# WoodOxen/tactics2d

Measured on NVIDIA H100. Metric: participant_steps_per_sec, higher is better.
Workload: dtype f32

## Files before the change

include/t2d_b200.h:

```cpp
#ifndef T2D_B200_H
#define T2D_B200_H

#include <stdint.h>

#ifdef __cplusplus
extern "C" {
#endif

#define T2D_VERSION 100

#define T2D_OK 0
#define T2D_E_INVALID (-1)
#define T2D_E_CUDA (-2)
#define T2D_E_UNSUPPORTED (-3)
#define T2D_E_STATE (-4)

#define T2D_MODEL_KINEMATICS 0
#define T2D_MODEL_DYNAMICS 1
#define T2D_MODEL_POINTMASS_NEWTON 2
#define T2D_MODEL_POINTMASS_EULER 3
#define T2D_MODEL_STATIC 4
#define T2D_MODEL_DRIFT 5

#define T2D_SHAPE_OBB 0
// ... 258 lines not shown
                        uint8_t* agent_status, float* iou, uint8_t* done, float* max_iou, float* min_dist,
                        uint8_t* traffic_status, int reset_trackers_on_done, void* stream);

int t2d_scatter_agent_action(t2d_ctx* ctx, const int16_t* observers , int32_t n_observers,
                             const float* agent_action , float* action ,
                             void* stream);
int t2d_step_host_agents(t2d_ctx* ctx, const float* agent_action_host , float* action ,
                         uint8_t* flags, int16_t* hit_index, int16_t* hit_segment, float* max_iou, float* min_dist,
                         int reset_trackers_on_done, float* reward_host, uint8_t* terminated_host, uint8_t* truncated_host,
                         uint8_t* agent_status_host, uint8_t* done_host, void* stream);

typedef struct t2d_exchange t2d_exchange;
int t2d_exchange_create(t2d_exchange** out, int device, int world, int rank, int n_local, int slots, void* ipc_handle_out);
int t2d_exchange_connect(t2d_exchange* x, const void* handles );
int t2d_exchange_allgather(t2d_exchange* x, const uint8_t* done_local, uint8_t* dst, void* stream);
int t2d_exchange_allgather_lagged(t2d_exchange* x, const uint8_t* done_local, uint8_t* dst, int lag, void* stream);
int t2d_exchange_status(t2d_exchange* x, uint32_t* steps, uint32_t* timed_out);
int t2d_exchange_destroy(t2d_exchange* x);

int t2d_physics_step(int device, const t2d_type_params* params , int interval_ms, int delta_t_ms, int n,
                     float* x, float* y, float* heading, float* speed, float* vx, float* vy, float* omega_front,
                     float* omega_rear, const float* action, float* applied, void* stream);

int t2d_set_prefetch(t2d_ctx* ctx, int mode);

int64_t t2d_launch_count(void);

int64_t t2d_tick_fixed_count(void);

int64_t t2d_tick_order_fallback_count(void);

int t2d_order_hint(t2d_ctx* ctx, void* read_to, const void* write_from);

int64_t t2d_tick_instance_count(int k);

#ifdef __cplusplus
}
#endif
#endif
```

tactics2d_b200/_lib.py:

```python

from __future__ import annotations

import ctypes as C
import os

_HERE = os.path.dirname(os.path.abspath(__file__))
LIB_PATH = os.environ.get("T2D_B200_LIB", os.path.join(_HERE, "libt2d_b200.so"))


class T2DError(RuntimeError):
    """A C-ABI call returned a negative code; the message is ``t2d_last_error()``."""


class Config(C.Structure):
    _fields_ = [("interval_ms", C.c_int32), ("delta_t_ms", C.c_int32), ("max_step", C.c_int32),
                ("flags", C.c_int32)]


class TypeParamsC(C.Structure):
    _fields_ = [(n, C.c_float) for n in (
        "half_len", "half_wid", "radius", "lf", "lr", "steer_lo", "steer_hi", "speed_lo", "speed_hi",
        "accel_lo", "accel_hi", "mass", "mass_height", "mu", "I_z", "cf", "cr")] + [
        ("model", C.c_int32), ("shape", C.c_int32)] + [(n, C.c_float) for n in ("wheel_radius", "T_sb", "T_se", "I_yw")]

# ... 81 lines not shown
    "t2d_bev_render_agents": (C.c_int, [_P, _P, C.c_int32, _P, C.c_int, C.c_int, _P, C.c_int, _P, _P]),
    "t2d_observe": (C.c_int, [_P, C.POINTER(ObsConfigC), _P, _P, _P, _P]),
    "t2d_observe_agents": (C.c_int, [_P, C.POINTER(ObsConfigC), _P, C.c_int32, _P, _P, _P, _P, _P]),
    "t2d_set_controllers": (C.c_int, [_P, _P, C.c_int, _P, _P, _P, _P]),
    "t2d_set_paths": (C.c_int, [_P, _P, _P, C.c_int]),
    "t2d_control": (C.c_int, [_P, _P, _P]),
    "t2d_set_pid": (C.c_int, [_P, _P, _P]),
    "t2d_set_leader_search": (C.c_int, [_P, C.c_double, C.c_double, _P, _P]),
    "t2d_find_leaders": (C.c_int, [_P, C.c_double, C.c_double, _P, _P, _P]),
    "t2d_set_lane_change": (C.c_int, [_P, _P, _P, _P, _P, _P, _P]),
    "t2d_set_routes": (C.c_int, [_P, _P, C.c_double, C.c_double, C.c_float]),
    "t2d_bind_route_trackers": (C.c_int, [_P, _P, _P, C.c_int32]),
    "t2d_route_observe": (C.c_int, [_P, _P, C.c_int32, C.c_int, C.c_float, _P, _P]),
    "t2d_set_history": (C.c_int, [_P, C.c_int32]),
    "t2d_observe_history": (C.c_int, [_P, _P, C.c_int32, _P, C.c_int32, _P, _P]),
    "t2d_history_view": (C.c_int, [_P, C.POINTER(HistoryRingC)]),
    "t2d_exchange_create": (C.c_int, [C.POINTER(_P), C.c_int, C.c_int, C.c_int, C.c_int, C.c_int, _P]),
    "t2d_exchange_connect": (C.c_int, [_P, _P]),
    "t2d_exchange_allgather": (C.c_int, [_P, _P, _P, _P]),
    "t2d_exchange_allgather_lagged": (C.c_int, [_P, _P, _P, C.c_int, _P]),
    "t2d_exchange_status": (C.c_int, [_P, C.POINTER(C.c_uint32), C.POINTER(C.c_uint32)]),
    "t2d_exchange_destroy": (C.c_int, [_P]),
    "t2d_physics_step": (C.c_int, [C.c_int, C.POINTER(TypeParamsC), C.c_int, C.c_int, C.c_int] + [_P] * 11),
    "t2d_bind_wheel_state": (C.c_int, [_P, _P, _P]),
    "t2d_bind_reset_wheel_pool": (C.c_int, [_P, _P, _P]),
    "t2d_set_log": (C.c_int, [_P, C.POINTER(LogC)]),
    "t2d_set_log_schedule": (C.c_int, [_P, C.POINTER(LogC), _P, _P, C.c_int32, _P]),
    "t2d_set_log_reactive": (C.c_int, [_P, C.POINTER(ReactiveReplayC)]),
    "t2d_set_prefetch": (C.c_int, [_P, C.c_int]),
    "t2d_launch_count": (C.c_int64, []),
    "t2d_tick_fixed_count": (C.c_int64, []),
    "t2d_tick_order_fallback_count": (C.c_int64, []),
    "t2d_order_hint": (C.c_int, [_P, _P, _P]),
    "t2d_tick_instance_count": (C.c_int64, [C.c_int]),
}

_lib = None


def load():
    global _lib
    if _lib is not None:
        return _lib
    if not os.path.exists(LIB_PATH):
        raise ImportError(
            f"{LIB_PATH} not found: build it with `python -c 'import __graft_entry__ as g; g.build()'` "
            "(nvcc -gencode arch=compute_90a,code=sm_90a).  tactics2d_b200 has no CPU fallback.")
    lib = C.CDLL(LIB_PATH)
    for name, (res, args) in SYMBOLS.items():
        fn = getattr(lib, name)
        fn.restype = res
        fn.argtypes = args
    _lib = lib
    return lib


def check(code: int):
    if code != 0:
        msg = load().t2d_last_error()
        raise T2DError(f"t2d error {code}: {msg.decode() if msg else ''}")
```

tactics2d_b200/csrc/t2d_kernels.cu:

```cuda
#include <cuda_runtime.h>
#include <stddef.h>
#include <stdint.h>
#include <stdio.h>
#include <string.h>

#include <algorithm>
#include <atomic>
#include <cmath>
#include <memory>
#include <mutex>
#include <string>
#include <vector>

#include "../../include/t2d_b200.h"
#include "t2d_math.cuh"
#include "t2d_world.cuh"
#include "t2d_tick.cuh"
#include "t2d_reset.cuh"
#include "t2d_route.cuh"
#include "t2d_agents.cuh"
#include "t2d_replay.cuh"
#include "t2d_lidar.cuh"
#include "t2d_exchange.cuh"
#include "t2d_control.cuh"
// ... 195 lines not shown
  float* ctrl_last_accel = nullptr;
  bool ctrl_has_pid = false;
  bool ctrl_pid_reads_target = false;
  const float* pid_target = nullptr;
  double* pid_state = nullptr;
  dev_ptr<PathVertex> d_path_v;
  dev_ptr<int> d_path_off;
  int n_paths = 0;
  int16_t* leader_lead = nullptr;
  float* leader_gap = nullptr;
  double leader_half_width = 0.0, leader_max_range = 0.0;
  std::unique_ptr<LaneChange> lane;
  std::unique_ptr<ReactiveReplay> reactive;
  const int16_t* route_id = nullptr;
  double route_threshold = 0.0, route_weight = 0.0;
  float route_off_reward = 0.0f;
  double* route_s_best = nullptr;
  double* route_agent_s_best = nullptr;
  int route_agent_rows = 0;
  std::unique_ptr<ChunkedUpload> hs_upload;
  Mirror hs_out;
  MappedEgo hs_ego;
  AgentStaging ha;
  dev_ptr<uint8_t> ha_flags;
  int host_chunks = 0;
  int n_bev_styles = 0;
  t2d_bev_style bev_style[bev::MAX_STYLES] = {};
  uint8_t bev_type_style[T2D_MAX_TYPES] = {};
  int bev_target_style = bev::NO_STYLE;
  std::unique_ptr<DeviceLog> log;
  std::vector<int> type_model;
  std::vector<t2d_type_params> type_rows;
  dev_ptr<uint8_t> order;
  std::unique_ptr<DeviceSampler> sampler;
  std::unique_ptr<DeviceHistory> hist;
};

enum : unsigned { NEED_STATE = 1, NEED_TABLE = 2, NEED_TICK = 4 };

static int require(const t2d_ctx* c, unsigned need) {
  if ((need & NEED_STATE) && !c->x) return fail(T2D_E_STATE, "state not bound: call t2d_bind_state first");
  if ((need & NEED_TABLE) && (!c->d_table || c->n_types == 0))
    return fail(T2D_E_STATE, "type table not set: call t2d_set_type_table first");
  if (need & NEED_TICK) {
    if (c->has_drift && !(c->wheel_f && c->wheel_r))
      return fail(T2D_E_STATE, "the type table holds a SingleTrackDrift row: call t2d_bind_wheel_state first");
    if (c->log && c->log->type_id != c->type_id) return fail(T2D_E_STATE, "state rebound after t2d_set_log: call t2d_set_log again");
  }
  return T2D_OK;
}

static WorldArgs world_args(const t2d_ctx* c) {
  return {c->x, c->y, c->h, c->v, c->vx, c->vy, c->type_id, c->step_count, c->d_table.get(), c->n_types, c->N, c->M};
}

static RouteArgs route_args(const t2d_ctx* c) {
  return {c->route_id, c->d_path_v.get(), c->d_path_off.get(), c->n_paths, c->route_off_reward, c->route_threshold,
          c->route_weight};
}

static int check_route_trackers(const t2d_ctx* c, const char* fn) {
  if (c->route_id && c->route_agent_s_best && c->route_agent_rows != c->agent_q)
    return fail(T2D_E_STATE, std::string(fn) + ": the agents' route tracker has another row count than the bound agents: "
                                               "call t2d_bind_route_trackers again");
  return T2D_OK;
}
// ... 42 lines not shown
  g_launches.fetch_add(1);
  CUDA_TRY(cudaGetLastError());
  return T2D_OK;
}

static int capped_grid(long long items, int per_cta, int sm_count, int per_sm) {
  return (int)std::max(1LL, std::min((items + per_cta - 1) / per_cta, (long long)sm_count * per_sm));
}

static int launch_history(t2d_ctx* c, const uint8_t* mask, void* stream) {
  if (!c->hist) return T2D_OK;
  hist::AppendArgs A{world_args(c)};
  A.ring = history_ring(c); A.track_now = history_track_now(c); A.mask = mask;
  hist::t2d_history_append_kernel<<<(c->N + hist::K15_WARPS - 1) / hist::K15_WARPS, hist::K15_WARPS * 32, 0, (cudaStream_t)stream>>>(A);
  return launched();
}

template <class Args> static void set_time_step(Args& A, int interval_ms, int delta_t_ms) {
  const int delta_t = std::min(delta_t_ms, interval_ms);
  A.n_steps = interval_ms / delta_t;
  A.dt = (float)((double)delta_t / 1000.0);
  A.dt_rem = (float)((double)(interval_ms % delta_t) / 1000.0);
  A.dt_d = (double)delta_t / 1000.0;
  A.dt_rem_d = (double)(interval_ms % delta_t) / 1000.0;
  A.interval_d = (double)interval_ms / 1000.0;
}

extern "C" {

int t2d_version(void) { return T2D_VERSION; }
const char* t2d_last_error(void) { return g_err.c_str(); }
int64_t t2d_launch_count(void) { return (int64_t)g_launches.load(); }
int64_t t2d_tick_fixed_count(void) { return (int64_t)(g_tick_instances[4].load() + g_tick_instances[5].load()); }
int64_t t2d_tick_order_fallback_count(void) {
  std::lock_guard<std::mutex> lock(g_order_mutex);
  int64_t sum = 0;
  for (unsigned long long* d : g_order_fallbacks) {
    if (!d) continue;
    unsigned long long n[ORDER_COUNTERS * ORDER_COUNTER_STRIDE];
    if (cudaMemcpy(n, d, sizeof(n), cudaMemcpyDeviceToHost) != cudaSuccess) return -1;
    for (int i = 0; i < ORDER_COUNTERS; ++i) sum += (int64_t)n[i * ORDER_COUNTER_STRIDE];
  }
  return sum;
}
int64_t t2d_tick_instance_count(int k) { return k >= 0 && k < 7 ? (int64_t)g_tick_instances[k].load() : -1; }

#ifdef T2D_TICK_TIMELINE
int t2d_tick_timeline(void* dst, int64_t bytes, int clear) {
  if (!dst || bytes != (int64_t)sizeof(t2d_timeline)) return fail(T2D_E_INVALID, "timeline buffer size");
  CUDA_TRY(cudaMemcpyFromSymbol(dst, t2d_timeline, sizeof(t2d_timeline)));
  if (clear) {
    void* p = nullptr;
    CUDA_TRY(cudaGetSymbolAddress(&p, t2d_timeline));
    CUDA_TRY(cudaMemset(p, 0, sizeof(t2d_timeline)));
  }
  return T2D_OK;
}
#endif

static int check_cfg(const t2d_config* cfg) {
  if (!cfg) return fail(T2D_E_INVALID, "cfg is NULL");
  if (cfg->interval_ms <= 0) return fail(T2D_E_INVALID, "interval_ms must be > 0");
  if (cfg->delta_t_ms <= 0) return fail(T2D_E_INVALID, "delta_t_ms must be > 0");
  return T2D_OK;
}

int t2d_create(t2d_ctx** out, int device, int n_scenarios, int m_participants, const t2d_config* cfg) {
  if (!out) return fail(T2D_E_INVALID, "out is NULL");
  *out = nullptr;
  if (int r = check_cfg(cfg)) return r;
  if (n_scenarios <= 0 || m_participants <= 0) return fail(T2D_E_INVALID, "n_scenarios and m_participants must be > 0");
  if (m_participants > T2D_MAX_PARTICIPANTS)
    return fail(T2D_E_UNSUPPORTED, "m_participants > 128: a scenario must fit one warp (4 participants per lane)");
  int count = 0;
  CUDA_TRY(cudaGetDeviceCount(&count));
  if (device < 0 || device >= count) return fail(T2D_E_INVALID, "no such CUDA device");
  CUDA_TRY(cudaSetDevice(device));
  t2d_ctx* c = new t2d_ctx();
  c->device = device;
  c->N = n_scenarios;
  c->M = m_participants;
  if (const char* e = getenv("T2D_PDL")) c->use_pdl = atoi(e) != 0;
  if (const char* e = getenv("T2D_GRID_LIMIT")) c->grid_limit = std::max(0, atoi(e));
  if (const char* e = getenv("T2D_TICK_GENERIC")) c->tick_generic = atoi(e) != 0;
  if (const char* e = getenv("T2D_PREFETCH")) c->prefetch_override = atoi(e) != 0 ? 1 : 0;
  if (const char* e = getenv("T2D_WPC")) {
    const int v = atoi(e);
    if (v >= 1 && v <= MAX_WARPS_PER_CTA) c->wpc_override = v;
  }
  if (const char* e = getenv("T2D_HOST_CHUNKS")) c->host_chunks = std::max(0, std::min(atoi(e), MAX_HOST_CHUNKS));
  int g = 1;
  while (g * PPL < m_participants) g <<= 1;
  c->G = g;
  c->cfg = *cfg;
  cudaDeviceProp prop;
  CUDA_TRY(cudaGetDeviceProperties(&prop, device));
  c->sm_count = prop.multiProcessorCount;
  c->max_smem_optin = (int)prop.sharedMemPerBlockOptin;
  {
    std::lock_guard<std::mutex> lock(g_order_mutex);
    unsigned long long*& counters = g_order_fallbacks[device % 64];
    const size_t bytes = ORDER_COUNTERS * ORDER_COUNTER_STRIDE * sizeof(unsigned long long);
    if (!counters && (cudaMalloc(&counters, bytes) != cudaSuccess || cudaMemset(counters, 0, bytes) != cudaSuccess)) {
      cudaFree(counters);
      counters = nullptr;
      delete c;
      return fail(T2D_E_CUDA, "t2d_create: cannot allocate the order fallback counters");
    }
  }
  {
    std::vector<uint8_t> identity((size_t)n_scenarios * FIX_M);
    for (size_t i = 0; i < identity.size(); ++i) identity[i] = (uint8_t)(i % FIX_M);
    if (int r = upload(c->order, identity.data(), identity.size())) {
      delete c;
      return r;
    }
  }
  *out = c;
  return T2D_OK;
}

int t2d_order_hint(t2d_ctx* c, void* read_to, const void* write_from) {
  if (!c) return fail(T2D_E_INVALID, "ctx is NULL");
  CUDA_TRY(cudaSetDevice(c->device));
  const size_t bytes = (size_t)c->N * FIX_M;
  if (read_to) CUDA_TRY(cudaMemcpy(read_to, c->order.get(), bytes, cudaMemcpyDeviceToHost));
  if (write_from) CUDA_TRY(cudaMemcpy(c->order.get(), write_from, bytes, cudaMemcpyHostToDevice));
  return T2D_OK;
}

int t2d_destroy(t2d_ctx* c) {
  if (!c) return T2D_OK;
  cudaSetDevice(c->device);
  delete c;
  return T2D_OK;
}

int t2d_set_config(t2d_ctx* c, const t2d_config* cfg) {
  if (!c) return fail(T2D_E_INVALID, "ctx is NULL");
  if (int r = check_cfg(cfg)) return r;
  c->cfg = *cfg;
  return T2D_OK;
}

int t2d_set_type_table(t2d_ctx* c, const t2d_type_params* table, int n_types) {
  if (!c || !table) return fail(T2D_E_INVALID, "ctx/table is NULL");
  if (n_types <= 0 || n_types > T2D_MAX_TYPES) return fail(T2D_E_INVALID, "n_types must be in 1..64");
  static_assert(sizeof(t2d_type_params) == sizeof(AbiParams), "type table layout");
  if (c->log)
    for (uint8_t row : c->log->track_type_host)
      if (row >= n_types || table[row].model != T2D_MODEL_STATIC)
        return fail(T2D_E_INVALID, "type table: row " + std::to_string(row) + " of a replayed track must exist and be T2D_MODEL_STATIC");
  bool has_pointmass = false, has_drift = false, kin_only = true;
  float rb_max = 0.0f;
  for (int i = 0; i < n_types; ++i) {
    const t2d_type_params& p = table[i];
    if (p.shape == T2D_SHAPE_OBB) rb_max = std::max(rb_max, sqrtf(p.half_len * p.half_len + p.half_wid * p.half_wid) * 1.000002f);
    if (p.shape == T2D_SHAPE_CIRCLE) rb_max = std::max(rb_max, p.radius);
    if (p.model < 0 || p.model > T2D_MODEL_DRIFT) return fail(T2D_E_INVALID, "type table: unknown model id");
    if (p.shape < 0 || p.shape > T2D_SHAPE_NONE) return fail(T2D_E_INVALID, "type table: unknown shape id");
// ... 438 lines not shown
  const int resident_warps = 14;
  if (tiles > (long long)sm_count * resident_warps) return MAX_WARPS_PER_CTA;
  int best = 2;
  double best_cost = 1e30;
  for (int w = 2; w <= MAX_WARPS_PER_CTA; ++w) {
    const long long ctas = (tiles + w - 1) / w;
    const long long per_sm = (ctas + sm_count - 1) / sm_count;
    const double cost = (double)(per_sm * w) + 0.42 * (double)per_sm;
    if (cost < best_cost - 1e-9 || (cost < best_cost + 1e-9 && w > best)) { best_cost = cost; best = w; }
  }
  return best;
}

static int launch_step(t2d_ctx* c, const float* action, const float* ego, uint8_t* flags, int16_t* hit_index, int16_t* hit_segment,
                       uint8_t* scn_status, uint8_t* done, void* stream, int do_physics, int first = 0, int count = -1) {
  if (!c) return fail(T2D_E_INVALID, "ctx is NULL");
  if (int r = require(c, NEED_STATE | NEED_TABLE)) return r;
  if (do_physics && !action) return fail(T2D_E_INVALID, "action is NULL");
  if (do_physics)
    if (int r = require(c, NEED_TICK)) return r;
  CUDA_TRY(cudaSetDevice(c->device));
  if (count < 0) count = c->N - first;
  if (first < 0 || count <= 0 || first + count > c->N) return fail(T2D_E_INVALID, "scenario range out of bounds");
  const DeviceMap& map = c->map;
  const size_t p0 = (size_t)first * c->M;
  StepArgs A{};
  A.x = c->x + p0; A.y = c->y + p0; A.h = c->h + p0; A.v = c->v + p0; A.vx = c->vx + p0; A.vy = c->vy + p0;
  A.type_id = c->type_id + p0; A.step_count = c->step_count + first;
  A.wheel_f = c->wheel_f ? c->wheel_f + p0 : nullptr; A.wheel_r = c->wheel_r ? c->wheel_r + p0 : nullptr;
  A.action = action; A.ego_action = ego ? ego + 2 * (size_t)first : nullptr; A.flags = flags; A.hit_index = hit_index; A.hit_segment = hit_segment;
  A.scn_status = scn_status; A.done = done;
  A.order = c->order.get() + (size_t)first * FIX_M;
  A.order_fallbacks = g_order_fallbacks[c->device % 64];
  const bool map_table = map.n_tiles > 1;
  const MapArgs mp = map_args(map, first);
  A.map_blob = mp.map_blob; A.tile_off = mp.tile_off; A.tile_id = mp.tile_id; A.map_bytes = map.smem_bytes; A.mh = map.mh;
  A.map_in_smem = (!map_table && map.blob && map.mh.n_seg > 0 && map.smem_bytes <= MAP_SMEM_LIMIT) ? 1 : 0;
  A.table = c->d_table.get(); A.n_types = c->n_types;
  A.N = count; A.M = c->M; A.G = c->G;
  set_time_step(A, c->cfg.interval_ms, c->cfg.delta_t_ms);
  A.max_step = c->cfg.max_step; A.cfg_flags = c->cfg.flags;
  A.do_physics = do_physics; A.has_bounds = map.has_bounds ? 1 : 0;
  A.bxmin = map.mh.bxmin; A.bxmax = map.mh.bxmax; A.bymin = map.mh.bymin; A.bymax = map.mh.bymax;
  A.prefetch = c->prefetch_override >= 0 ? c->prefetch_override : (g_exchanges_alive.load() == 0 ? 1 : 0);
  A.needs_vel_in = (c->has_pointmass || c->has_drift || (do_physics && c->log)) ? 1 : 0;
  bool vec = (c->M % PPL == 0) && aligned16(A.x) && aligned16(A.y) && aligned16(A.h) && aligned16(A.v) && aligned16(A.vx) &&
             aligned16(A.vy) && aligned4(A.type_id) && aligned16(action) && aligned4(flags) && aligned8(hit_index) &&
             aligned8(hit_segment);
  A.vec_ok = vec ? 1 : 0;

  A.rb_max = c->rb_max;
  A.goal = c->goal;
  if (A.goal.target) {
    A.goal.target += 5 * (size_t)first; A.goal.iou += first; A.goal.last_pose += 4 * (size_t)first; A.goal.noact_count += first;
  }
  const int table_bytes = (((c->n_types + 1) * (int)sizeof(Params) + 15) / 16) * 16;
  const int spw = 32 / c->G;
  const long long tiles = ((long long)count + spw - 1) / spw;
  int wpc = pick_wpc(tiles, c->sm_count);
  if (c->wpc_override > 0) wpc = c->wpc_override;
  {
    int off = (A.map_in_smem ? A.map_bytes : 0) + table_bytes;
    A.off_poseA = off; off += wpc * POSE_PER_WARP * (int)sizeof(float4);
    A.off_poseB = off; off += wpc * POSE_PER_WARP * (int)sizeof(float4);
    A.off_hit = off; off += wpc * POSE_PER_WARP * (int)sizeof(int);
    A.off_queue = off; off += wpc * QCAP * 4;
// ... 1141 lines not shown
```

tactics2d_b200/csrc/t2d_math.cuh:

```cuda
#pragma once

#include <math.h>
#include <string.h>
#include <stdint.h>

#if defined(__CUDACC__)
#define T2D_HD __host__ __device__ __forceinline__
#define T2D_HD_NOINLINE __host__ __device__ __noinline__
#else
#define T2D_HD inline
#define T2D_HD_NOINLINE
#endif

#if defined(__CUDA_ARCH__)
#define T2D_RSQRTF(x) rsqrtf(x)
#else
#define T2D_RSQRTF(x) (1.0f / sqrtf(x))
#endif

namespace t2d {

constexpr int MODEL_KINEMATICS = 0;
constexpr int MODEL_DYNAMICS = 1;
constexpr int MODEL_POINTMASS_NEWTON = 2;
// ... 144 lines not shown
  float x[W], y[W], h[W], v[W];
  float vx[W], vy[W];
  float ch[W], sh[W];
  float acc[W], steer[W];
};

template <int W>
T2D_HD void kinematics_finish(KinIO<W>& io, const Params* const (&p)[W], const float (&c)[W], const float (&s)[W], float (&v)[W],
                              const float (&Sx)[W], const float (&Sy)[W], const float (&Sv)[W], const float (&kdt)[W],
                              const float (&k)[W], const float (&a)[W], const float (&vlo)[W], const float (&vhi)[W], float dt,
                              float dt_rem) {
#pragma unroll
  for (int i = 0; i < W; ++i) {
    float x = fmaf(dt, Sx[i], io.x[i]);
    float y = fmaf(dt, Sy[i], io.y[i]);
    float dphi = kdt[i] * Sv[i];
    if (dt_rem > 0.0f) {
      x = fmaf(dt_rem * v[i], c[i], x);
      y = fmaf(dt_rem * v[i], s[i], y);
      dphi = fmaf(k[i] * dt_rem, v[i], dphi);
      v[i] = clampf(fmaf(a[i], dt_rem, v[i]), vlo[i], vhi[i]);
    }
    float hn = wrap_two_pi(io.h[i] + dphi);
    float sh, ch;
    sincos_core(hn, sh, ch);
    io.x[i] = x; io.y[i] = y; io.h[i] = hn; io.v[i] = v[i];
    io.vx[i] = v[i] * ch;
    io.vy[i] = v[i] * sh;
    io.ch[i] = ch; io.sh[i] = sh;
  }
}

template <int W>
T2D_HD void kinematics_step(KinIO<W>& io, const Params* const (&p)[W], int n_steps, float dt, float dt_rem) {
  float c[W], s[W], w1[W], Sx[W], Sy[W], Sv[W], kdt[W], adt[W], vlo[W], vhi[W], k[W], a[W];
  bool small = true;
  bool lin = n_steps >= 2 && n_steps <= 24;
  float sd[W], cd[W], sp[W], cp[W];
  bool rare = false;
#pragma unroll
  for (int i = 0; i < W; ++i) {
    const Vec4 g0 = params_group(p[i], 0);
    a[i] = clampf(io.acc[i], g0.x, g0.y);
    const float d = clampf(io.steer[i], g0.z, g0.w);
    io.acc[i] = a[i];
    io.steer[i] = d;
    sincos_poly(d, sd[i], cd[i]);
    sincos_core(io.h[i], sp[i], cp[i]);
    rare = rare || !(fabsf(d) <= 0.78f) || !(fabsf(io.h[i]) <= 512.0f);
  }
  if (rare) {
#pragma unroll
    for (int i = 0; i < W; ++i) {
      if (!(fabsf(io.steer[i]) <= 0.78f)) sincos_fast(io.steer[i], &sd[i], &cd[i]);
      if (!(fabsf(io.h[i]) <= 512.0f)) sincos_fast(io.h[i], &sp[i], &cp[i]);
    }
  }
#pragma unroll
  for (int i = 0; i < W; ++i) {
    const Vec4 g1 = params_group(p[i], 1);
    const float tan_d = T2D_FDIV(sd[i], cd[i]);
    const float tb = g1.z * tan_d;
    const float cb = T2D_RSQRTF(fmaf(tb, tb, 1.0f));
    const float sb = tb * cb;
    k[i] = tan_d * cb * g1.w;
    kdt[i] = k[i] * dt;
    adt[i] = a[i] * dt;
    c[i] = cp[i] * cb - sp[i] * sb;
    s[i] = sp[i] * cb + cp[i] * sb;
    vlo[i] = g1.x;
    vhi[i] = g1.y;
    const float w1u = fmaf(a[i], dt, io.v[i]);
    w1[i] = clampf(w1u, vlo[i], vhi[i]);
    const float wlu = fmaf((float)(n_steps - 1), adt[i], w1[i]);
    const float wl = clampf(fmaf((float)(n_steps - 2), adt[i], w1[i]), vlo[i], vhi[i]);
    lin = lin && (w1u == w1[i]) && (wlu >= vlo[i]) && (wlu <= vhi[i]) && (fabsf(kdt[i] * adt[i]) <= 1e-4f);
    const float wmax = fmaxf(fabsf(io.v[i]), fmaxf(fabsf(w1[i]), fabsf(wl)));
    small = small && (fabsf(kdt[i]) * wmax <= 0.25f);
    Sx[i] = 0.0f; Sy[i] = 0.0f; Sv[i] = 0.0f;
  }
#if defined(__CUDA_ARCH__)
  const bool fast = __all_sync(__activemask(), lin && small);
// ... 622 lines not shown
```

tactics2d_b200/csrc/t2d_tick.cuh:

```cuda
#pragma once

#include "t2d_world.cuh"

namespace t2d {

struct StepArgs {
  float *x, *y, *h, *v, *vx, *vy;
  const uint8_t* type_id;
  int32_t* step_count;
  const float* action;
  const float* ego_action;
  uint8_t* flags;
  int16_t* hit_index;
  int16_t* hit_segment;
  uint8_t* scn_status;
  uint8_t* done;
  const unsigned char* map_blob;
  const uint32_t* tile_off;
  const uint16_t* tile_id;
  MapHeader mh;
  const Params* table;
  int map_bytes, map_in_smem;
  int n_types;
  int N, M, G;
  int g_shift, mp_shift, unused1, n_tiles, wpc, table_bytes;
  int off_poseA, off_poseB, off_hit, off_queue, off_sorted, unused0, off_qcount, off_bar;
  int n_steps;
  float dt, dt_rem;
  double dt_d, dt_rem_d, interval_d;
  int max_step, cfg_flags;
  int do_physics, has_bounds, vec_ok, needs_vel_in;
  int prefetch;
  float bxmin, bxmax, bymin, bymax;
  float rb_max;
  GoalArgs goal;
  float *wheel_f, *wheel_r;
  uint8_t* order;
  unsigned long long* order_fallbacks;
};

__device__ __noinline__ void other_model_step(OneIO& io, const Params& p, int n_steps, double dt, double dt_rem, double interval) {
  if (p.model() == MODEL_DYNAMICS) {
    dynamics_step(io, p, n_steps, dt);
  } else if (p.model() == MODEL_POINTMASS_NEWTON) {
    pointmass_newton_step(io, p, interval);
  } else if (p.model() == MODEL_POINTMASS_EULER) {
    pointmass_euler_step(io, p, n_steps, dt, dt_rem);
  } else {
    sincos_fast(io.h, &io.sh, &io.ch);
  }
}

__device__ __forceinline__ unsigned near_fetch(const float ax, const float ay, const float rbound, const MapHeader& mh, const uint8_t* fine,
                                               unsigned& alt) {
  const float r = rbound * 1.0001f + 1e-3f;
  const float fx = (ax - mh.x0) * mh.inv_cell, fy = (ay - mh.y0) * mh.inv_cell;
  const float gxf = (float)mh.gx, gyf = (float)mh.gy;
  const bool inside = fx >= 0.0f && fy >= 0.0f && fx < gxf && fy < gyf;
  const float kf = (float)mh.fine;
  const int nx = mh.gx * mh.fine, ny = mh.gy * mh.fine;
  const float ux = fmaf(inside ? fx : 0.0f, kf, -0.5f), uy = fmaf(inside ? fy : 0.0f, kf, -0.5f);
  int ix = __float_as_int(ux + RINT_MAGIC) - 0x4B400000, iy = __float_as_int(uy + RINT_MAGIC) - 0x4B400000;
  ix = min(max(ix, 0), nx - 1); iy = min(max(iy, 0), ny - 1);
  const unsigned q = (unsigned)__ldg(fine + (size_t)iy * nx + ix);
  const float ox = fmaxf(fmaxf(-fx, fx - gxf), 0.0f), oy = fmaxf(fmaxf(-fy, fy - gyf), 0.0f);
  const unsigned q_out = fmaxf(ox, oy) * mh.cell <= r ? 0u : 255u;
  alt = inside ? 0xffffffffu : q_out;
  return q;
}
__device__ __forceinline__ bool near_decide(unsigned q, unsigned alt, const float rbound) {
  const unsigned v = alt == 0xffffffffu ? q : alt;
// ... 157 lines not shown
      const MapView mv = map_view(t.sec, *t.mh);
      *sm = static_walk_exact(load_pose(poseA, poseB, ti), poseA[pslot(ti)].z, *t.mh, mv.seg, mv.cell_start, mv.items);
    }
    if (t.mh->n_poly > 0) {
      const float4 pa = poseA[pslot(ti)];
      *sm = static_objects(*sm, pa.x, pa.y, *t.mh, t.blob);
    }
  }
  __syncwarp();
}

__device__ __noinline__ bool oob_slow(const float4* poseA, const float4* poseB, int idx, float xmin, float xmax, float ymin, float ymax) {
  const Pose a = load_pose(poseA, poseB, idx);
  int r = out_of_bound_f32(a.x, a.y, a.c, a.s, a.l, a.w, a.w < 0.0f, xmin, xmax, ymin, ymax);
  if (r < 0) r = out_of_bound_f64(a.x, a.y, a.h, a.l, a.w, a.w < 0.0f, xmin, xmax, ymin, ymax) ? 1 : 0;
  return r != 0;
}

constexpr int FIX_M = 64, FIX_G = 16, FIX_G_SHIFT = 4, FIX_MP_SHIFT = 6;

constexpr int COHORT_BAR = 1;
__device__ __forceinline__ void cohort_arrive(int threads) {
  asm volatile("barrier.arrive %0, %1;" ::"n"(COHORT_BAR), "r"(threads) : "memory");
}
__device__ __forceinline__ void cohort_wait(int threads) {
  asm volatile("barrier.sync %0, %1;" ::"n"(COHORT_BAR), "r"(threads) : "memory");
}

#ifndef T2D_ORDER_PASSES
#define T2D_ORDER_PASSES 2
#endif
constexpr int ORDER_COUNTERS = 64, ORDER_COUNTER_STRIDE = 16;

template <bool FIXED>
__device__ __forceinline__ void prefetch_tile_l2(const StepArgs& A, long long i) {
  asm volatile("prefetch.global.L2 [%0];" ::"l"(A.x + i));
  asm volatile("prefetch.global.L2 [%0];" ::"l"(A.y + i));
  asm volatile("prefetch.global.L2 [%0];" ::"l"(A.h + i));
  asm volatile("prefetch.global.L2 [%0];" ::"l"(A.v + i));
  if (FIXED || A.action) asm volatile("prefetch.global.L2 [%0];" ::"l"(A.action + 2 * i));
  asm volatile("prefetch.global.L2 [%0];" ::"l"(A.type_id + i));
  if (FIXED) asm volatile("prefetch.global.L2 [%0];" ::"l"(A.order + i));
  if (!FIXED && A.needs_vel_in) {
    asm volatile("prefetch.global.L2 [%0];" ::"l"(A.vx + i));
    asm volatile("prefetch.global.L2 [%0];" ::"l"(A.vy + i));
  }
}

#ifdef T2D_TICK_TIMELINE
constexpr int TL_POINTS = 9, TL_MAX_WARPS = 4096;
__device__ unsigned long long t2d_timeline[TL_MAX_WARPS][TL_POINTS][2];
#define T2D_TL(k, on, slot, dep)                                                                                    \
  do {                                                                                                              \
    if ((on) && (slot) < TL_MAX_WARPS) {                                                                            \
      unsigned long long g_, c_;                                                                                    \
      asm volatile("mov.u64 %0, %%globaltimer;\n\tmov.u64 %1, %%clock64;" : "=l"(g_), "=l"(c_) : "f"(dep) : "memory"); \
      t2d_timeline[slot][k][0] = g_;                                                                                \
      t2d_timeline[slot][k][1] = c_;                                                                                \
    }                                                                                                               \
  } while (0)
#else
#define T2D_TL(k, on, slot, dep)
#endif

template <bool KIN_ONLY, bool MAP_TABLE, bool FIXED>
__global__ void __launch_bounds__(CTA_THREADS, 2) t2d_step_kernel(const __grid_constant__ StepArgs A) {
  extern __shared__ __align__(128) unsigned char smem[];
  T2D_TL(0, (threadIdx.x & 31) == 0, (int)(blockIdx.x * A.wpc + (threadIdx.x >> 5)), 0.0f);
  const int map_smem_bytes = (!MAP_TABLE && A.map_in_smem) ? A.map_bytes : 0;
  const int table_bytes = A.table_bytes;
  const int wpc = A.wpc;
  unsigned char* s_map = smem;
  Params* s_table = reinterpret_cast<Params*>(smem + map_smem_bytes);
  float4* s_poseA = reinterpret_cast<float4*>(smem + A.off_poseA);
  float4* s_poseB = reinterpret_cast<float4*>(smem + A.off_poseB);
// ... 36 lines not shown
  float4* poseA = s_poseA + warp * POSE_PER_WARP;
  float4* poseB = s_poseB + warp * POSE_PER_WARP;
  int* hitmin = s_hit + warp * POSE_PER_WARP;
  unsigned* queue = s_queue + warp * QCAP;
  int* qcount = s_qcount + warp;
  const int tb = sub * MP, t0 = tb + m0;
  const int mp_shift = K1_SHAPE(mp_shift, FIX_MP_SHIFT);
  float4* sorted = s_sorted + warp * POSE_PER_WARP + tb;
  const int Mh = M >> 1;

  const int n_tiles = A.n_tiles;
  const int tile0 = (int)blockIdx.x * wpc + warp;
  if (cohort_b) cohort_wait(wpc * 32);
  else if (cohorts && tile0 >= n_tiles) cohort_arrive(wpc * 32);
  for (int tile = tile0; tile < n_tiles; tile += (int)gridDim.x * wpc) {
    const long long n = (long long)tile * spw + sub;
    const bool scn_ok = n < A.N;
    int nvalid = scn_ok ? (FIXED ? PPL : min(PPL, M - m0)) : 0;
    if (nvalid < 0) nvalid = 0;
    const long long idx0 = n * M + m0;
#ifdef T2D_TICK_TIMELINE
    const bool tl_on = lane == 0 && tile == (int)blockIdx.x * wpc + warp;
    const int tl_slot = tile;
#endif

    float sx[PPL], sy[PPL], shd[PPL], sv[PPL], svx[PPL], svy[PPL], a0[PPL], a1[PPL];
    int tidv[PPL];
#pragma unroll
    for (int i = 0; i < PPL; ++i) {
      sx[i] = sy[i] = shd[i] = sv[i] = svx[i] = svy[i] = a0[i] = a1[i] = 0.0f;
      tidv[i] = T2D_TYPE_INACTIVE;
    }
    uint32_t hint = 0x03020100u + 0x04040404u * (uint32_t)gl;
    if (nvalid == PPL && K1_SHAPE(vec_ok, 1)) {
      ld_vec<float, PPL>(A.x + idx0, sx);
      ld_vec<float, PPL>(A.y + idx0, sy);
      ld_vec<float, PPL>(A.h + idx0, shd);
      ld_vec<float, PPL>(A.v + idx0, sv);
      uint8_t tb8[PPL];
      ld_vec<uint8_t, PPL>(A.type_id + idx0, tb8);
      if constexpr (FIXED) hint = *reinterpret_cast<const uint32_t*>(A.order + idx0);
#pragma unroll
      for (int i = 0; i < PPL; ++i) tidv[i] = tb8[i];
      if (K1_SHAPE(do_physics, 1)) {
        float2 act[PPL];
        float lo[4], hi[4];
        ld_vec<float, 4>(A.action + 2 * idx0, lo);
        ld_vec<float, 4>(A.action + 2 * idx0 + 4, hi);
        act[0] = make_float2(lo[0], lo[1]); act[1] = make_float2(lo[2], lo[3]);
        act[2] = make_float2(hi[0], hi[1]); act[3] = make_float2(hi[2], hi[3]);
#pragma unroll
        for (int i = 0; i < PPL; ++i) { a0[i] = act[i].x; a1[i] = act[i].y; }
        if (K1_SHAPE(needs_vel_in, 0)) {
          ld_vec<float, PPL>(A.vx + idx0, svx);
          ld_vec<float, PPL>(A.vy + idx0, svy);
        }
      }
    } else {
#pragma unroll
      for (int i = 0; i < PPL; ++i) {
        if (i < nvalid) {
          sx[i] = A.x[idx0 + i]; sy[i] = A.y[idx0 + i]; shd[i] = A.h[idx0 + i]; sv[i] = A.v[idx0 + i];
          tidv[i] = A.type_id[idx0 + i];
          if (K1_SHAPE(do_physics, 1)) {
            a0[i] = A.action[2 * (idx0 + i)]; a1[i] = A.action[2 * (idx0 + i) + 1];
            if (K1_SHAPE(needs_vel_in, 0)) { svx[i] = A.vx[idx0 + i]; svy[i] = A.vy[idx0 + i]; }
          }
        }
      }
    }
    if (cohorts && !cohort_b && tile == tile0) cohort_arrive(wpc * 32);
    {
      const long long n_next = n + (long long)gridDim.x * wpc * spw;
      if (A.prefetch && n_next < A.N && m0 < M) prefetch_tile_l2<FIXED>(A, n_next * M + m0);
// ... 10 lines not shown
    bool active[PPL], kin[PPL];
    const Params* pp[PPL];
    int model[PPL];
    bool lane_all_kin = true, lane_any_kin = false;
#pragma unroll
    for (int i = 0; i < PPL; ++i) {
      active[i] = tidv[i] < A.n_types;
      pp[i] = &s_table[active[i] ? tidv[i] : 0];
      model[i] = pp[i]->model_shape & 0xff;
      kin[i] = active[i] && (model[i] == MODEL_KINEMATICS);
      lane_all_kin = lane_all_kin && kin[i];
      lane_any_kin = lane_any_kin || kin[i];
      ch[i] = 1.0f; sh[i] = 0.0f;
    }
    T2D_TL(2, tl_on, tl_slot, sx[PPL - 1] + sy[PPL - 1] + shd[PPL - 1] + sv[PPL - 1] + a0[PPL - 1] + a1[PPL - 1] + (float)model[PPL - 1]);
    if (A.cfg_flags & T2D_CFG_STEER_FIRST) {
#pragma unroll
      for (int i = 0; i < PPL; ++i)
        if (model[i] <= MODEL_DYNAMICS || model[i] == MODEL_DRIFT) { float t = a0[i]; a0[i] = a1[i]; a1[i] = t; }
    }

    if (K1_SHAPE(do_physics, 1)) {
      if (__any_sync(0xffffffffu, lane_any_kin)) {
        const Params* const null_row = &s_table[A.n_types];
        const Params* pk[PPL];
        KinIO<PPL> io;
#pragma unroll
        for (int i = 0; i < PPL; ++i) {
          pk[i] = kin[i] ? pp[i] : null_row;
          io.x[i] = kin[i] ? sx[i] : 0.0f; io.y[i] = kin[i] ? sy[i] : 0.0f;
          io.h[i] = kin[i] ? shd[i] : 0.0f; io.v[i] = kin[i] ? sv[i] : 0.0f;
          io.acc[i] = kin[i] ? a0[i] : 0.0f; io.steer[i] = kin[i] ? a1[i] : 0.0f;
        }
        kinematics_step<PPL>(io, pk, A.n_steps, A.dt, A.dt_rem);
#pragma unroll
        for (int i = 0; i < PPL; ++i) {
          if (kin[i]) {
            sx[i] = io.x[i]; sy[i] = io.y[i]; shd[i] = io.h[i]; sv[i] = io.v[i];
            svx[i] = io.vx[i]; svy[i] = io.vy[i]; ch[i] = io.ch[i]; sh[i] = io.sh[i];
          }
        }
      }
      if (!lane_all_kin) {
#pragma unroll
        for (int i = 0; i < PPL; ++i) {
          if (active[i] && !kin[i]) {
            if constexpr (!KIN_ONLY) {
              OneIO io;
              io.x = sx[i]; io.y = sy[i]; io.h = shd[i]; io.v = sv[i]; io.vx = svx[i]; io.vy = svy[i];
              io.a0 = a0[i]; io.a1 = a1[i];
              io.ch = 1.0f; io.sh = 0.0f;
              other_model_step(io, *pp[i], A.n_steps, A.dt_d, A.dt_rem_d, A.interval_d);
              sx[i] = io.x; sy[i] = io.y; shd[i] = io.h; sv[i] = io.v; svx[i] = io.vx; svy[i] = io.vy;
              ch[i] = io.ch; sh[i] = io.sh;
            } else {
              sincos_fast(shd[i], &sh[i], &ch[i]);
            }
          }
        }
      }
      bool all_active = true;
#pragma unroll
      for (int i = 0; i < PPL; ++i) all_active = all_active && active[i];
      if (nvalid == PPL && K1_SHAPE(vec_ok, 1) && all_active) {
        st_vec<float, PPL>(A.x + idx0, sx);
        st_vec<float, PPL>(A.y + idx0, sy);
        st_vec<float, PPL>(A.h + idx0, shd);
        st_vec<float, PPL>(A.v + idx0, sv);
        st_vec<float, PPL>(A.vx + idx0, svx);
        st_vec<float, PPL>(A.vy + idx0, svy);
      } else {
#pragma unroll
        for (int i = 0; i < PPL; ++i) {
          if (i < nvalid && active[i]) {
            A.x[idx0 + i] = sx[i]; A.y[idx0 + i] = sy[i]; A.h[idx0 + i] = shd[i]; A.v[idx0 + i] = sv[i];
            A.vx[idx0 + i] = svx[i]; A.vy[idx0 + i] = svy[i];
          }
        }
      }
    } else {
#pragma unroll
      for (int i = 0; i < PPL; ++i) sincos_fast(shd[i], &sh[i], &ch[i]);
    }
    T2D_TL(3, tl_on, tl_slot, sx[0] + sy[PPL - 1] + ch[0] + sh[PPL - 1]);

    float px[PPL], py[PPL], rb[PPL];
    unsigned solid_bits = 0;
#pragma unroll
    for (int i = 0; i < PPL; ++i) {
      const Vec4 g2 = params_group(pp[i], 2);
      const bool sol = active[i] && (__float_as_int(g2.w) >> 8) != SHAPE_NONE;
      solid_bits |= sol ? (1u << i) : 0u;
      rb[i] = g2.z;
      px[i] = sol ? sx[i] : __int_as_float(0x7fc00000);
      py[i] = sy[i];
      poseA[i * 32 + lane] = make_float4(px[i], py[i], rb[i], shd[i]);
      poseB[i * 32 + lane] = make_float4(ch[i], sh[i], g2.x, g2.y);
    }
    if (lane == 0) *qcount = 0;
    __syncwarp();
    const int cnt_in = (K1_SHAPE(do_physics, 1) && gl == 0 && scn_ok) ? A.step_count[n] : 0;

    unsigned near_q[PPL], near_alt[PPL];
#pragma unroll
    for (int i = 0; i < PPL; ++i) { near_q[i] = 255u; near_alt[i] = 255u; }
    const MapHeader* lane_mh = &A.mh;
    const unsigned char* lane_blob = A.map_blob;
    if constexpr (MAP_TABLE) {
      lane_blob = A.map_blob + A.tile_off[scn_ok ? A.tile_id[n] : 0];
// ... 302 lines not shown
```

Baseline: 17.40 billion.

## Cache heading cos/sin across ticks to skip trig on step entry

Adds a per-participant device cache of cos/sin of heading, tagged with the heading value it was computed for, to the fixed-M world. The kinematic step reuses the cached values when the tag matches the current heading and falls back to sincos per lane on a miss, counting misses in a new counter. This is meant to remove one sincos per participant per tick, at the cost of three extra float loads and three extra stores per participant, plus L2 prefetches for them.

```diff
diff --git a/include/t2d_b200.h b/include/t2d_b200.h
--- a/include/t2d_b200.h
+++ b/include/t2d_b200.h
@@ -314,6 +314,10 @@
 
 int t2d_order_hint(t2d_ctx* ctx, void* read_to, const void* write_from);
 
+int64_t t2d_tick_trig_fallback_count(void);
+
+int t2d_heading_trig(t2d_ctx* ctx, void* read_to, const void* write_from);
+
 int64_t t2d_tick_instance_count(int k);
 
 #ifdef __cplusplus
diff --git a/tactics2d_b200/_lib.py b/tactics2d_b200/_lib.py
--- a/tactics2d_b200/_lib.py
+++ b/tactics2d_b200/_lib.py
@@ -137,6 +137,8 @@
     "t2d_tick_fixed_count": (C.c_int64, []),
     "t2d_tick_order_fallback_count": (C.c_int64, []),
     "t2d_order_hint": (C.c_int, [_P, _P, _P]),
+    "t2d_tick_trig_fallback_count": (C.c_int64, []),
+    "t2d_heading_trig": (C.c_int, [_P, _P, _P]),
     "t2d_tick_instance_count": (C.c_int64, [C.c_int]),
 }
 
diff --git a/tactics2d_b200/csrc/t2d_kernels.cu b/tactics2d_b200/csrc/t2d_kernels.cu
--- a/tactics2d_b200/csrc/t2d_kernels.cu
+++ b/tactics2d_b200/csrc/t2d_kernels.cu
@@ -251,6 +251,7 @@
   std::vector<int> type_model;
   std::vector<t2d_type_params> type_rows;
   dev_ptr<uint8_t> order;
+  dev_ptr<float> trig;
   std::unique_ptr<DeviceSampler> sampler;
   std::unique_ptr<DeviceHistory> hist;
 };
@@ -359,17 +360,19 @@
 const char* t2d_last_error(void) { return g_err.c_str(); }
 int64_t t2d_launch_count(void) { return (int64_t)g_launches.load(); }
 int64_t t2d_tick_fixed_count(void) { return (int64_t)(g_tick_instances[4].load() + g_tick_instances[5].load()); }
-int64_t t2d_tick_order_fallback_count(void) {
+static int64_t fixed_fallback_sum(int set) {
   std::lock_guard<std::mutex> lock(g_order_mutex);
   int64_t sum = 0;
   for (unsigned long long* d : g_order_fallbacks) {
     if (!d) continue;
     unsigned long long n[ORDER_COUNTERS * ORDER_COUNTER_STRIDE];
-    if (cudaMemcpy(n, d, sizeof(n), cudaMemcpyDeviceToHost) != cudaSuccess) return -1;
+    if (cudaMemcpy(n, d + set * ORDER_COUNTERS * ORDER_COUNTER_STRIDE, sizeof(n), cudaMemcpyDeviceToHost) != cudaSuccess) return -1;
     for (int i = 0; i < ORDER_COUNTERS; ++i) sum += (int64_t)n[i * ORDER_COUNTER_STRIDE];
   }
   return sum;
 }
+int64_t t2d_tick_order_fallback_count(void) { return fixed_fallback_sum(0); }
+int64_t t2d_tick_trig_fallback_count(void) { return fixed_fallback_sum(1); }
 int64_t t2d_tick_instance_count(int k) { return k >= 0 && k < 7 ? (int64_t)g_tick_instances[k].load() : -1; }
 
 #ifdef T2D_TICK_TIMELINE
@@ -427,7 +430,7 @@
   {
     std::lock_guard<std::mutex> lock(g_order_mutex);
     unsigned long long*& counters = g_order_fallbacks[device % 64];
-    const size_t bytes = ORDER_COUNTERS * ORDER_COUNTER_STRIDE * sizeof(unsigned long long);
+    const size_t bytes = 2 * ORDER_COUNTERS * ORDER_COUNTER_STRIDE * sizeof(unsigned long long);
     if (!counters && (cudaMalloc(&counters, bytes) != cudaSuccess || cudaMemset(counters, 0, bytes) != cudaSuccess)) {
       cudaFree(counters);
       counters = nullptr;
@@ -443,6 +446,15 @@
       return r;
     }
   }
+  if (m_participants == FIX_M) {
+    const size_t plane = (size_t)n_scenarios * FIX_M;
+    std::vector<float> trig(3 * plane, 0.0f);
+    std::fill(trig.begin(), trig.begin() + plane, 1.0f);
+    if (int r = upload(c->trig, trig.data(), trig.size())) {
+      delete c;
+      return r;
+    }
+  }
   *out = c;
   return T2D_OK;
 }
@@ -453,6 +465,16 @@
   const size_t bytes = (size_t)c->N * FIX_M;
   if (read_to) CUDA_TRY(cudaMemcpy(read_to, c->order.get(), bytes, cudaMemcpyDeviceToHost));
   if (write_from) CUDA_TRY(cudaMemcpy(c->order.get(), write_from, bytes, cudaMemcpyHostToDevice));
+  return T2D_OK;
+}
+
+int t2d_heading_trig(t2d_ctx* c, void* read_to, const void* write_from) {
+  if (!c) return fail(T2D_E_INVALID, "ctx is NULL");
+  if (!c->trig) return fail(T2D_E_UNSUPPORTED, "t2d_heading_trig: the world has no heading trig cache (M != 64)");
+  CUDA_TRY(cudaSetDevice(c->device));
+  const size_t bytes = 3 * (size_t)c->N * FIX_M * sizeof(float);
+  if (read_to) CUDA_TRY(cudaMemcpy(read_to, c->trig.get(), bytes, cudaMemcpyDeviceToHost));
+  if (write_from) CUDA_TRY(cudaMemcpy(c->trig.get(), write_from, bytes, cudaMemcpyHostToDevice));
   return T2D_OK;
 }
 
@@ -957,6 +979,11 @@
   A.scn_status = scn_status; A.done = done;
   A.order = c->order.get() + (size_t)first * FIX_M;
   A.order_fallbacks = g_order_fallbacks[c->device % 64];
+  if (c->trig) {
+    const size_t plane = (size_t)c->N * FIX_M, f0 = (size_t)first * FIX_M;
+    A.trig_c = c->trig.get() + f0; A.trig_s = c->trig.get() + plane + f0; A.trig_tag = c->trig.get() + 2 * plane + f0;
+  }
+  A.trig_fallbacks = A.order_fallbacks + ORDER_COUNTERS * ORDER_COUNTER_STRIDE;
   const bool map_table = map.n_tiles > 1;
   const MapArgs mp = map_args(map, first);
   A.map_blob = mp.map_blob; A.tile_off = mp.tile_off; A.tile_id = mp.tile_id; A.map_bytes = map.smem_bytes; A.mh = map.mh;
diff --git a/tactics2d_b200/csrc/t2d_math.cuh b/tactics2d_b200/csrc/t2d_math.cuh
--- a/tactics2d_b200/csrc/t2d_math.cuh
+++ b/tactics2d_b200/csrc/t2d_math.cuh
@@ -200,7 +200,14 @@
 }
 
 template <int W>
-T2D_HD void kinematics_step(KinIO<W>& io, const Params* const (&p)[W], int n_steps, float dt, float dt_rem) {
+struct HeadingTrig {
+  unsigned ok;
+  float c[W], s[W];
+};
+
+template <int W, bool TRIG_IN = false>
+T2D_HD void kinematics_step(KinIO<W>& io, const Params* const (&p)[W], int n_steps, float dt, float dt_rem,
+                            const HeadingTrig<W>* trig = nullptr) {
   float c[W], s[W], w1[W], Sx[W], Sy[W], Sv[W], kdt[W], adt[W], vlo[W], vhi[W], k[W], a[W];
   bool small = true;
   bool lin = n_steps >= 2 && n_steps <= 24;
@@ -214,8 +221,23 @@
     io.acc[i] = a[i];
     io.steer[i] = d;
     sincos_poly(d, sd[i], cd[i]);
-    sincos_core(io.h[i], sp[i], cp[i]);
+    if constexpr (TRIG_IN) {
+      sp[i] = trig->s[i];
+      cp[i] = trig->c[i];
+    } else {
+      sincos_core(io.h[i], sp[i], cp[i]);
+    }
     rare = rare || !(fabsf(d) <= 0.78f) || !(fabsf(io.h[i]) <= 512.0f);
+  }
+  if constexpr (TRIG_IN) {
+    if (trig->ok != (1u << W) - 1u) {
+#pragma unroll
+      for (int i = 0; i < W; ++i) {
+        float si, ci;
+        sincos_core(io.h[i], si, ci);
+        if (!((trig->ok >> i) & 1u)) { sp[i] = si; cp[i] = ci; }
+      }
+    }
   }
   if (rare) {
 #pragma unroll
diff --git a/tactics2d_b200/csrc/t2d_tick.cuh b/tactics2d_b200/csrc/t2d_tick.cuh
--- a/tactics2d_b200/csrc/t2d_tick.cuh
+++ b/tactics2d_b200/csrc/t2d_tick.cuh
@@ -37,6 +37,8 @@
   float *wheel_f, *wheel_r;
   uint8_t* order;
   unsigned long long* order_fallbacks;
+  float *trig_c, *trig_s, *trig_tag;
+  unsigned long long* trig_fallbacks;
 };
 
 __device__ __noinline__ void other_model_step(OneIO& io, const Params& p, int n_steps, double dt, double dt_rem, double interval) {
@@ -260,6 +262,14 @@
 #endif
 constexpr int ORDER_COUNTERS = 64, ORDER_COUNTER_STRIDE = 16;
 
+
+#ifndef T2D_TRIG_CACHE
+#define T2D_TRIG_CACHE 1
+#endif
+#ifndef T2D_TRIG_PREFETCH
+#define T2D_TRIG_PREFETCH 1
+#endif
+
 template <bool FIXED>
 __device__ __forceinline__ void prefetch_tile_l2(const StepArgs& A, long long i) {
   asm volatile("prefetch.global.L2 [%0];" ::"l"(A.x + i));
@@ -268,7 +278,14 @@
   asm volatile("prefetch.global.L2 [%0];" ::"l"(A.v + i));
   if (FIXED || A.action) asm volatile("prefetch.global.L2 [%0];" ::"l"(A.action + 2 * i));
   asm volatile("prefetch.global.L2 [%0];" ::"l"(A.type_id + i));
-  if (FIXED) asm volatile("prefetch.global.L2 [%0];" ::"l"(A.order + i));
+  if (FIXED) {
+    asm volatile("prefetch.global.L2 [%0];" ::"l"(A.order + i));
+    if (T2D_TRIG_CACHE && T2D_TRIG_PREFETCH) {
+      asm volatile("prefetch.global.L2 [%0];" ::"l"(A.trig_c + i));
+      asm volatile("prefetch.global.L2 [%0];" ::"l"(A.trig_s + i));
+      asm volatile("prefetch.global.L2 [%0];" ::"l"(A.trig_tag + i));
+    }
+  }
   if (!FIXED && A.needs_vel_in) {
     asm volatile("prefetch.global.L2 [%0];" ::"l"(A.vx + i));
     asm volatile("prefetch.global.L2 [%0];" ::"l"(A.vy + i));
@@ -371,6 +388,9 @@
       tidv[i] = T2D_TYPE_INACTIVE;
     }
     uint32_t hint = 0x03020100u + 0x04040404u * (uint32_t)gl;
+    float tc[PPL], ts[PPL], ttag[PPL];
+#pragma unroll
+    for (int i = 0; i < PPL; ++i) tc[i] = ts[i] = ttag[i] = 0.0f;
     if (nvalid == PPL && K1_SHAPE(vec_ok, 1)) {
       ld_vec<float, PPL>(A.x + idx0, sx);
       ld_vec<float, PPL>(A.y + idx0, sy);
@@ -378,7 +398,14 @@
       ld_vec<float, PPL>(A.v + idx0, sv);
       uint8_t tb8[PPL];
       ld_vec<uint8_t, PPL>(A.type_id + idx0, tb8);
-      if constexpr (FIXED) hint = *reinterpret_cast<const uint32_t*>(A.order + idx0);
+      if constexpr (FIXED) {
+        hint = *reinterpret_cast<const uint32_t*>(A.order + idx0);
+        if (T2D_TRIG_CACHE) {
+          ld_vec<float, PPL>(A.trig_c + idx0, tc);
+          ld_vec<float, PPL>(A.trig_s + idx0, ts);
+          ld_vec<float, PPL>(A.trig_tag + idx0, ttag);
+        }
+      }
 #pragma unroll
       for (int i = 0; i < PPL; ++i) tidv[i] = tb8[i];
       if (K1_SHAPE(do_physics, 1)) {
@@ -455,7 +482,24 @@
           io.h[i] = kin[i] ? shd[i] : 0.0f; io.v[i] = kin[i] ? sv[i] : 0.0f;
           io.acc[i] = kin[i] ? a0[i] : 0.0f; io.steer[i] = kin[i] ? a1[i] : 0.0f;
         }
-        kinematics_step<PPL>(io, pk, A.n_steps, A.dt, A.dt_rem);
+        if constexpr (FIXED && T2D_TRIG_CACHE) {
+          HeadingTrig<PPL> trig;
+          unsigned miss = 0;
+#pragma unroll
+          for (int i = 0; i < PPL; ++i) {
+            trig.c[i] = tc[i];
+            trig.s[i] = ts[i];
+            if (kin[i] && __float_as_uint(ttag[i]) != __float_as_uint(shd[i])) miss |= 1u << i;
+          }
+          trig.ok = ~miss & ((1u << PPL) - 1u);
+          kinematics_step<PPL, true>(io, pk, A.n_steps, A.dt, A.dt_rem, &trig);
+          if (__any_sync(0xffffffffu, miss != 0)) {
+            const unsigned evaluated = __reduce_add_sync(0xffffffffu, (unsigned)__popc(miss));
+            if (lane == 0) atomicAdd(&A.trig_fallbacks[(blockIdx.x & (ORDER_COUNTERS - 1)) * ORDER_COUNTER_STRIDE], (unsigned long long)evaluated);
+          }
+        } else {
+          kinematics_step<PPL>(io, pk, A.n_steps, A.dt, A.dt_rem);
+        }
 #pragma unroll
         for (int i = 0; i < PPL; ++i) {
           if (kin[i]) {
@@ -492,12 +536,18 @@
         st_vec<float, PPL>(A.v + idx0, sv);
         st_vec<float, PPL>(A.vx + idx0, svx);
         st_vec<float, PPL>(A.vy + idx0, svy);
+        if constexpr (FIXED && T2D_TRIG_CACHE) {
+          st_vec<float, PPL>(A.trig_c + idx0, ch);
+          st_vec<float, PPL>(A.trig_s + idx0, sh);
+          st_vec<float, PPL>(A.trig_tag + idx0, shd);
+        }
       } else {
 #pragma unroll
         for (int i = 0; i < PPL; ++i) {
           if (i < nvalid && active[i]) {
             A.x[idx0 + i] = sx[i]; A.y[idx0 + i] = sy[i]; A.h[idx0 + i] = shd[i]; A.v[idx0 + i] = sv[i];
             A.vx[idx0 + i] = svx[i]; A.vy[idx0 + i] = svy[i];
+            if constexpr (FIXED && T2D_TRIG_CACHE) { A.trig_c[idx0 + i] = ch[i]; A.trig_s[idx0 + i] = sh[i]; A.trig_tag[idx0 + i] = shd[i]; }
           }
         }
       }
```

Measured after the change: 15.67 billion (median of 6 runs). 10.0% lower.
